# TU-Delft-AI-Energy-Lab/Deep-Statistical-Solver-for-Distribution-System-State-Estimation

Hardware: AMD Instinct MI355X
Metric: grid-samples/sec fwd+bwd (WLS loss), CIGRE-14 batch=4096, 1/2/4/8 GPU (higher is better)
Workload: dtype f32 (H->H products as f16x3: two fp16 pieces per operand, 3 fp16 MFMAs per fp32 product, f32 accumulate; edge MLP bf16x6; everything else f32/f64); 1 GPU; CIGRE-14 (15 buses, 14 closed branches) B=4096 graphs/GPU, MPN L=4 H=128 K=2 dropout=0: forward + gsp_wls_edge + backward; graphs_per_gpu=4096, global_batch=4096, parallelism=dp1, ranks_seen=1, arithmetic_route=f16x3, plan_launches=9, clock_ramp_steps_before_warmup=5740, mode=launch plan (dss2_plan_run)

## Files before the change

### deep-statistical-solver-for-distribution-system-state-estimation_amd/_lib.py

```python
from __future__ import annotations

import ctypes as C
import os
import subprocess

_HERE = os.path.dirname(os.path.abspath(__file__))
LIB_PATH = os.environ.get("DSS2_LIB", os.path.join(_HERE, "libdss2_hip.so"))

c_f32p = C.c_void_p
c_i32p = C.c_void_p


class PackDesc(C.Structure):
    _fields_ = [("src", C.c_void_p), ("dst", C.c_void_p), ("rows", C.c_int32), ("cols", C.c_int32),
                ("ld", C.c_int32), ("transpose", C.c_int32), ("koff", C.c_int32), ("kpad", C.c_int32),
                ("ncg", C.c_int32), ("joff", C.c_int32)]


class GemmPropArgs(C.Structure):
    _fields_ = [("X", C.c_void_p), ("ldx", C.c_int64), ("kreal", C.c_int32), ("kpad", C.c_int32),
                ("Bp", C.c_void_p), ("bias", C.c_void_p), ("rowscale", C.c_void_p),
                ("relu_src", C.c_void_p), ("ld_relu", C.c_int64),
                ("dmask", C.c_void_p), ("ld_dmask", C.c_int64),
                ("add_src", C.c_void_p), ("ld_add", C.c_int64),
# ... 280 lines not shown
    "dss2_wgrad": (C.c_int, [C.POINTER(WgradArgs), C.c_void_p]),
    "dss2_wgrad_batched": (C.c_int, [C.c_void_p, C.c_void_p, C.c_void_p, C.c_void_p, C.c_void_p, C.c_int64, C.c_int, C.c_void_p]),
    "dss2_reduce_slabs_multi": (C.c_int, [C.c_void_p, C.c_int, C.c_void_p]),
    "dss2_reduce_slabs": (C.c_int, [C.c_void_p, C.c_int, C.c_int64, C.c_void_p, C.c_int64, C.c_void_p]),
    "dss2_wls_loss_partials": (C.c_int, [C.POINTER(WlsArgs), C.c_void_p]),
    "dss2_wls_loss_grad": (C.c_int, [C.POINTER(WlsArgs), C.c_void_p]),
    "dss2_wls_loss_value": (C.c_int, [C.POINTER(WlsArgs), C.c_void_p]),
    "dss2_get_pflow": (C.c_int, [C.c_void_p, C.c_int64, C.c_void_p, C.c_int64, C.c_void_p, C.c_int64,
                                 C.c_void_p, C.c_void_p, C.c_int64, C.c_int64, C.c_void_p, C.c_void_p,
                                 C.c_int, C.c_void_p]),
    "dss2_eval_batch": (C.c_int, [C.c_void_p, C.c_int64, C.c_void_p, C.c_int64, C.c_void_p, C.c_int64, C.c_void_p, C.c_int64,
                                  C.c_void_p, C.c_void_p, C.c_int64, C.c_int64, C.c_void_p, C.c_void_p, C.c_void_p,
                                  C.c_void_p, C.c_void_p, C.c_void_p, C.c_void_p, C.c_void_p, C.c_void_p]),
    "dss2_eval_scratch_doubles": (C.c_int64, []),
    "dss2_small_gemm": (C.c_int, [C.c_void_p, C.c_int, C.c_int, C.c_void_p, C.c_void_p]),
    "dss2_measure_nodes": (C.c_int, [C.c_void_p, C.c_void_p, C.c_int32, C.c_void_p, C.c_double, C.c_double, C.c_double,
                                     C.c_double, C.c_void_p, C.c_int64, C.c_void_p]),
    "dss2_measure_edges": (C.c_int, [C.c_void_p, C.c_void_p, C.c_int32, C.c_void_p, C.c_double, C.c_void_p, C.c_int64,
                                     C.c_void_p]),
    "dss2_masked_zscore": (C.c_int, [C.c_void_p, C.c_int64, C.c_int32, C.c_int32, C.c_void_p, C.c_int32, C.c_void_p,
                                     C.c_void_p, C.c_void_p, C.c_void_p]),
    "dss2_masked_zscore_scratch_doubles": (C.c_int64, [C.c_int64]),
    "dss2_collate": (C.c_int, [C.c_void_p, C.c_int32, C.c_void_p, C.c_int64, C.c_void_p]),
    "dss2_csr_build_graphs": (C.c_int, [C.c_void_p, C.c_int32, C.c_void_p, C.c_int32, C.c_int32, C.c_void_p, C.c_void_p]),
    "dss2_csr_build_graphs_supported": (C.c_int, [C.c_int32, C.c_int32]),
    "dss2_csr_build_padded": (C.c_int, [C.POINTER(PaddedBuildArgs), C.c_void_p]),
    "dss2_collate_cursor": (C.c_int, [C.c_void_p, C.c_int32, C.c_void_p, C.c_void_p, C.c_int64, C.c_int, C.c_void_p]),
    "dss2_accum_scalar": (C.c_int, [C.c_void_p, C.c_void_p, C.c_void_p]),
    "dss2_collate_ragged_multi": (C.c_int, [C.c_void_p, C.c_int32, C.c_int32, C.c_void_p, C.c_void_p, C.c_void_p, C.c_void_p, C.c_int64, C.c_void_p]),
    "dss2_collate_ragged": (C.c_int, [C.c_void_p, C.c_int32, C.c_void_p, C.c_void_p, C.c_void_p, C.c_int64, C.c_int64, C.c_void_p]),
# ... 83 lines not shown
```

### deep-statistical-solver-for-distribution-system-state-estimation_amd/csrc/dss2_gemm_prop.hip

```cpp
#include <stdlib.h>

#include "dss2_weightspace.hpp"

namespace dss2 {

__global__ void __launch_bounds__(256) pack_weights_kernel(const dss2_pack_desc* __restrict__ descs) {
  pack_weights_body(descs[blockIdx.y], (int)blockIdx.x);
}

#ifdef DSS2_STAMPS
__device__ unsigned long long g_stamps[8192 * 8];
#define DSS2_STAMP(slot)                                                                       \
  do {                                                                                         \
    unsigned long long t_;                                                                     \
    __builtin_amdgcn_sched_barrier(0);                                                         \
    asm volatile("s_memtime %0\n\ts_waitcnt lgkmcnt(0)" : "=s"(t_)::"memory");                 \
    __builtin_amdgcn_sched_barrier(0);                                                         \
    if (lane == 0 && (stamp_tile * 4 + wave) < 8192) g_stamps[(stamp_tile * 4 + wave) * 8 + (slot)] = t_; \
  } while (0)
#define DSS2_STAMP2(slot)                                                                      \
  do {                                                                                         \
    unsigned long long t_;                                                                     \
    __builtin_amdgcn_sched_barrier(0);                                                         \
    asm volatile("s_memtime %0\n\ts_waitcnt lgkmcnt(0)" : "=s"(t_)::"memory");                 \
// ... 841 lines not shown

extern "C" size_t dss2_gemm_prop_lds_bytes(int nrb, int nmat, int kpad, int ncg, int max_nnz, int ell_width) {
  return dss2::lds_bytes(nrb, nmat, kpad, ncg, max_nnz, ell_width);
}

extern "C" int dss2_gemm_prop16_supported(int nrb, int nmat, int kreal, int hout, int max_nnz, int ell_width) {
  if (!((nrb == 6 && (nmat == 3 || nmat == 4)) || (nrb == 4 && nmat == 4))) return 0;
  return dss2::gemm16_shape_ok(nrb, nmat, kreal, hout, max_nnz, ell_width) ? 1 : 0;
}

static int dss2_pack_weights_launch(const dss2_pack_desc* descs, int n_desc, int max_elems, void* stream);
extern "C" int dss2_pack_weights(const dss2_pack_desc* descs, int n_desc, int max_elems, void* stream) {
  DSS2_RECORD([descs, n_desc, max_elems](void* s_) { return dss2_pack_weights_launch(descs, n_desc, max_elems, s_); });
  return dss2_pack_weights_launch(descs, n_desc, max_elems, stream);
}
static int dss2_pack_weights_launch(const dss2_pack_desc* descs, int n_desc, int max_elems, void* stream) {
  if (n_desc <= 0) return 0;
  dim3 grid((max_elems + 255) / 256, n_desc);
  hipLaunchKernelGGL(dss2::pack_weights_kernel, grid, dim3(256), 0, dss2::as_stream(stream), descs);
  return dss2::check_launch("pack_weights");
}

static int dss2_gemm_prop_launch(const dss2_gemm_prop_args* ap, void* stream);
extern "C" int dss2_gemm_prop(const dss2_gemm_prop_args* ap, void* stream) {
  if (!ap) { dss2::set_error("dss2_gemm_prop: null argument"); return 2; }
  DSS2_RECORD([a = *ap](void* s_) { return dss2_gemm_prop_launch(&a, s_); });
  return dss2_gemm_prop_launch(ap, stream);
}
static int dss2_gemm_prop_launch(const dss2_gemm_prop_args* ap, void* stream) {
  using namespace dss2;
// ... 63 lines not shown
```

### deep-statistical-solver-for-distribution-system-state-estimation_amd/csrc/dss2_weightspace.hpp

```cpp
#pragma once
#include "dss2_common.hpp"

namespace dss2 {

template <bool COH>
__device__ __forceinline__ void ws_store(float* p, float v) {
  if (COH) __hip_atomic_store((__attribute__((address_space(1))) float*)p, v, __ATOMIC_RELAXED, __HIP_MEMORY_SCOPE_AGENT);
  else *p = v;
}
template <bool COH>
__device__ __forceinline__ void ws_store4(float* p, f32x4 v) {
  if (COH) asm volatile("global_store_dwordx4 %0, %1, off sc1" ::"v"(p), "v"(v) : "memory");
  else *reinterpret_cast<f32x4*>(p) = v;
}

constexpr int SG_T = 32, SG_KC = 128, SG_LDA = SG_KC + 4;
template <bool tA, bool tB, bool COH = false, int NBUF = 3>
__device__ __forceinline__ void small_gemm_body(const dss2_sgemm_desc* __restrict__ dp, float* base_out,
                                                float (&As)[SG_T][SG_LDA], float (&Bs)[SG_KC][SG_T + 1], const int tile) {
  const int M = dp->M, N = dp->N, K = dp->K, lda = dp->lda, ldb = dp->ldb, ldc = dp->ldc;
  const bool accum = dp->accumulate != 0;
  const int nbatch = dp->nbatch;
  const float* u = dp->u;
  const float* v = dp->v;
  float* C = dp->c_off >= 0 ? base_out + dp->c_off : dp->C;
  const int tn = (N + SG_T - 1) / SG_T, tm = (M + SG_T - 1) / SG_T;
  if (tile >= tm * tn) return;
  const int i0 = (tile / tn) * SG_T, j0 = (tile % tn) * SG_T;
  const int t = threadIdx.x, lo = t & 31, hi = t >> 5;
  const int kchunks = (K + SG_KC - 1) / SG_KC;
  const int nchunks = nbatch * kchunks;
  float rab[NBUF][16], rbb[NBUF][16];
  auto issue = [&](int c, float (&ra)[16], float (&rb)[16]) {
    const int bidx = c / kchunks, k0 = (c - bidx * kchunks) * SG_KC;
    typedef const __attribute__((address_space(1))) float* gptr;
    const gptr A = (gptr)dp->A[bidx];
    const gptr B = (gptr)dp->B[bidx];
#pragma unroll
    for (int q = 0; q < 16; ++q) {
      const int i = tA ? lo : hi + 8 * (q >> 2), k = tA ? hi + 8 * q : lo + 32 * (q & 3);
      const int gi = min(i0 + i, M - 1), gk = min(k0 + k, K - 1);
      const float av = tA ? A[(size_t)gk * lda + gi] : A[(size_t)gi * lda + gk];
      ra[q] = av * (((i0 + i) < M && (k0 + k) < K) ? 1.f : 0.f);
      const int kb = tB ? lo + 32 * (q & 3) : hi + 8 * q, j = tB ? hi + 8 * (q >> 2) : lo;
      const int gj = min(j0 + j, N - 1), gkb = min(k0 + kb, K - 1);
      const float bv = tB ? B[(size_t)gj * ldb + gkb] : B[(size_t)gkb * ldb + gj];
      rb[q] = bv * (((j0 + j) < N && (k0 + kb) < K) ? 1.f : 0.f);
    }
// ... 20 lines not shown
      __syncthreads();
      stage(rab[u3], rbb[u3]);
      __syncthreads();
      if (c + NBUF < nchunks) issue(c + NBUF, rab[u3], rbb[u3]);
      const int kw = wave * 32;
#pragma unroll
      for (int g = 0; g < 8; ++g) {
        const f32x4 av = *reinterpret_cast<const f32x4*>(&As[c32][kw + 4 * g]);
#pragma unroll
        for (int tt = 0; tt < 2; ++tt) {
          const float a = half ? av[2 * tt + 1] : av[2 * tt];
          const float bvv = Bs[kw + 4 * g + 2 * tt + half][c32];
          acc = __builtin_amdgcn_mfma_f32_32x32x2f32(a, bvv, acc, 0, 0, 0);
        }
      }
    }
  }
  __syncthreads();
  float* red = &As[0][0];
#pragma unroll
  for (int r = 0; r < 16; ++r) red[(wave * 16 + r) * 64 + lane] = acc[r];
  __syncthreads();
  const int j = j0 + c32;
  if (j < N) {
    const float vj = u ? v[j] : 0.f;
#pragma unroll
    for (int q = 0; q < 4; ++q) {
      const int r = 4 * wave + q;
      const int i = i0 + (r & 3) + 8 * (r >> 2) + 4 * half;
      if (i >= M) continue;
      float sum = (red[(0 * 16 + r) * 64 + lane] + red[(1 * 16 + r) * 64 + lane]) + (red[(2 * 16 + r) * 64 + lane] + red[(3 * 16 + r) * 64 + lane]);
      if (u) sum = fmaf(u[i], vj, sum);
      float* cp = C + (size_t)i * ldc + j;
      ws_store<COH>(cp, accum ? *cp + sum : sum);
    }
  }
}

template <bool COH = false, int NBUF = 3>
__device__ __forceinline__ void small_gemm_tile(const dss2_sgemm_desc* __restrict__ dp, float* base_out,
                                                float (&As)[SG_T][SG_LDA], float (&Bs)[SG_KC][SG_T + 1], const int tile) {
  const bool ta = dp->transA != 0, tb = dp->transB != 0;
  if (ta) { if (tb) small_gemm_body<true, true, COH, NBUF>(dp, base_out, As, Bs, tile); else small_gemm_body<true, false, COH, NBUF>(dp, base_out, As, Bs, tile); }
  else    { if (tb) small_gemm_body<false, true, COH, NBUF>(dp, base_out, As, Bs, tile); else small_gemm_body<false, false, COH, NBUF>(dp, base_out, As, Bs, tile); }
}

__device__ __forceinline__ void pack_weights_body(const dss2_pack_desc d, const int bx) {
  const bool tr = d.transpose & 1;
  const int K = tr ? d.cols : d.rows;
  const int J = tr ? d.rows : d.cols;
  if (d.transpose & 8) {
    const int nkk = d.kpad >> 4, ncg = d.ncg;
    const int units = 2 * nkk;
    int U = 2; while (U < units) U <<= 1;
    if (U > 256) return;
    const int cpb = 256 / U;
    const int jpad = ncg * 32;
    if (bx * cpb >= jpad) return;
    __shared__ float cmx[256];
    typedef const __attribute__((address_space(1))) float* gsrc_t;
    const gsrc_t src = (gsrc_t)d.src;
    const int t = threadIdx.x, u = t & (U - 1), cj = t / U;
    const int j = bx * cpb + cj, kg = u >> 1, hf = u & 1;
    const bool active = u < units && j < jpad;
    float v[8];
    float mx = 0.f;
#pragma unroll
    for (int q = 0; q < 8; ++q) {
      const int k = kg * 16 + 8 * hf + q;
      const int kc = k >= K ? K - 1 : k, jc = j >= J ? J - 1 : j;
      const float x = tr ? src[(size_t)jc * d.ld + kc] : src[(size_t)kc * d.ld + jc];
      v[q] = (active && k < K && j < J) ? x : 0.f;
      mx = fmaxf(mx, fabsf(v[q]));
    }
// ... 58 lines not shown
  const int idx = bx * 256 + (int)threadIdx.x;
  if (idx >= total) return;
  const int lane = idx & 63;
  const int kg = kg0 + (idx >> 6) % nkl;
  const int cg = cg0 + (idx >> 6) / nkl;
  const int j = cg * 32 + (lane & 31) - d.joff;
  if (j < 0 || j >= J) return;
  float* dst = d.dst + (((size_t)cg * nkk + kg) * 64 + lane) * 4;
#pragma unroll
  for (int s = 0; s < 4; ++s) {
    const int k = kg * 8 + 4 * (lane >> 5) + s - d.koff;
    if (k >= 0 && k < K) dst[s] = tr ? d.src[(size_t)j * d.ld + k] : d.src[(size_t)k * d.ld + j];
  }
}


constexpr int REDUCE_MAX_DESC = 32;
struct ReduceTable { dss2_reduce_desc d[REDUCE_MAX_DESC]; uint32_t scalar_mask; };
__host__ __device__ __forceinline__ bool reduce_tall(const dss2_reduce_desc& d) { return d.n_slabs >= 256 && d.len <= 8192; }
__host__ __device__ __forceinline__ int64_t reduce_blocks(const dss2_reduce_desc& d, bool scalar) {
  return (!scalar && reduce_tall(d)) ? (d.len + 15) / 16 : (d.len + 63) / 64;
}
template <bool COH = false>
__device__ __forceinline__ void reduce_slabs_body(const dss2_reduce_desc& d, const bool scalar, const int bx, f32x4 (&part)[16][16]) {
  if (!scalar && reduce_tall(d)) {
    if ((int64_t)bx * 16 >= d.len) return;
    const int tid = threadIdx.x, cl = tid & 3, sl = tid >> 2;
    const int64_t i4 = (int64_t)bx * 16 + cl * 4;
    f32x4 s = {0.f, 0.f, 0.f, 0.f};
    f32x4* pt = &part[0][0];
// ... 88 lines not shown
```

### deep-statistical-solver-for-distribution-system-state-estimation_amd/flags.py

```python
import os as _os

EDGE_TILE_KERNELS = _os.environ.get("DSS2_EDGE_TILE", "1") == "1"
CHAIN_LAYERS = _os.environ.get("DSS2_CHAIN", "1") == "1"
WGRAD_BF16 = _os.environ.get("DSS2_WGRAD_BF16", "1") == "1"
CHAIN_GATE_BITS = _os.environ.get("DSS2_CHAIN_GATE_BITS", "1") == "1"
CHAIN_BF16 = _os.environ.get("DSS2_CHAIN_BF16", "1") == "1"
CHAIN_F16 = _os.environ.get("DSS2_CHAIN_F16", "1") == "1"
CHAIN_HEAD = _os.environ.get("DSS2_CHAIN_HEAD", "1") == "1"
CHAIN_HEAD_WGRAD = _os.environ.get("DSS2_CHAIN_HEAD_WGRAD", "1") == "1"
CHAIN_HEAD_FWD = _os.environ.get("DSS2_CHAIN_HEAD_FWD", "1") == "1"
CHAIN_EDGE = _os.environ.get("DSS2_CHAIN_EDGE", "1") == "1"
WGRAD_BATCH = _os.environ.get("DSS2_WGRAD_BATCH", "1") == "1"
STACK_NODE = _os.environ.get("DSS2_STACK_NODE", "1") == "1"
DX_MERGE = _os.environ.get("DSS2_DX_MERGE", "1") == "1"
WGRAD_JOIN_FOLDED = None
FOLD_W2 = _os.environ.get("DSS2_FOLD_W2", "1") == "1"
WGRAD_F16 = _os.environ.get("DSS2_WGRAD_F16", "1") == "1"
WGRAD_HOPS_MFMA = _os.environ.get("DSS2_WGRAD_HOPS_MFMA", "1") == "1"
WLS_FUSED_FINISH = _os.environ.get("DSS2_WLS_FUSED_FINISH", "0") == "1"
WLS_FUSED_FINISH_SMALL = _os.environ.get("DSS2_WLS_FUSED_FINISH_SMALL", "1") == "1"
WGRAD_TM32 = _os.environ.get("DSS2_WGRAD_TM32", "1") == "1"
WGRAD_TM32_MAX_BYTES = 64 << 20
WGRAD_PER_CU = int(_os.environ.get("DSS2_WGRAD_PER_CU", "2"))
CHAIN_MAX = 8
```

### deep-statistical-solver-for-distribution-system-state-estimation_amd/networks.py

```python
from __future__ import annotations

import ctypes as C
import os as _os
from typing import List, NamedTuple, Optional, Sequence, Tuple

import numpy as np
import torch
import torch.nn as nn

from . import _lib
from .topology import Topology, get_topology

_F32 = torch.float32

from . import flags as FL
from .ops import (_DROP_PARAMS, _dropout_params, _ncg, _ptr, _reduce, _require_gpu, _round16, _round8, _rows, _stream, _wgrad_per_cu, _wgrad_tiles, chain16_supported, chain_f16_supported, chain_gate_words, chain_edge_supported, chain_head_supported, chain_head_wgrad_supported, chain_supported, csr_axpy, dropout_mask, dropout_snapshot, edge_hidden_bwd, edge_hidden_fwd, edge_tile_bwd, edge_tile_fwd, gather_rows, gemm16_supported, gemm_prop, gemm_prop_chain, is_narrow, finish_weights, prep_weights, reduce_pending, segment_sum, wgrad, wgrad_batched)
from .plans import (_DESC_DTYPE, _FoldPlan, _MatView, _PackPlan, _SG_DTYPE, _as_view, _pack_table, _sg, _sg_table, _small_gemm)
from .route import BlockRoute, block_route, use_global_path


def _edge_aggr_forward(topo, x, ldx, ea, ldea, W1, b1, b2, pack_w2_fwd, hid, hout, fn, fe, second_linear=True, need_dx=False):
    N, ts = topo.N, topo.tiling
    S = torch.empty(N, hid, dtype=_F32, device=W1.device)
    if ts.ell_ent_tiles is not None and FL.EDGE_TILE_KERNELS:
        edge_tile_fwd(ts, x, ldx, ea, ldea, W1, b1, S, hid, fn, fe, need_dx)
    else:
        edge_hidden_fwd(topo, x, ldx, ea, ldea, W1, b1, S, hid, fn, fe)
    if not second_linear:
        return S, None
    x0 = torch.empty(N, hout, dtype=_F32, device=W1.device)
    gemm_prop(topo, S, hid, hid, pack_w2_fwd, 1, hout, x0, bias=b2, rowscale=topo.deg)
    return S, x0

# ... 488 lines not shown
    ver: int
    act_bits: dict


def _mpn_forward(mod, topo, x, ea, ps, stack=None, need_dx=False):
    x, ldx = _rows(x)
    ea, ldea = _rows(ea)
    dev = x.device
    L, nmat, hid = mod.n_gnn_layers, mod.K + 1, mod.dim_hid
    W1, b1, W2, b2 = ps[0:4]
    conv_ps = mod._conv_params(ps)
    rt = block_route(mod, topo, need_dx, False) if stack is None else stack.route_of(mod)
    ntiles = topo.tiling.ntiles
    plan, fold = _ensure_plans(mod, topo, dev, ps, rt)
    if stack is None:
        ver = plan.refresh(fold)
    else:
        ver = plan.version
    if not rt.glob:
        topo.lds_check(nmat, _round8(hid), _ncg(hid))
    if rt.edge:
        S = h = torch.empty(topo.N, hid, dtype=_F32, device=dev)
    else:
        S, h = _edge_aggr_forward(topo, x, ldx, ea, ldea, W1, b1, b2, plan.fwd[0], hid, hid, mod.dim_featn, mod.dim_feate,
                                  second_linear=fold is None, need_dx=need_dx)
    if fold is not None:
        h = S
    acts = [h]
    act_bits = {}
    p = float(mod.dropout_rate)
    if p <= 0.0:
# ... 203 lines not shown
        return (dx, None, None, None, *grads)


class _StackPlan:

    DROP_STRIDE = 64

    def __init__(self, blocks, device):
        self.blocks, self.device = list(blocks), device
        sizes = [int(m._flat_offsets()[-1]) for m in self.blocks]
        self.base = [0]
        for s in sizes:
            self.base.append(self.base[-1] + s)
        self.total = self.base[-1]
        self.key = None
        self.fold_fwd = self.fold_bwd = self.pack_tab = None
        self.table_builds = 0

    def refresh(self, topo, params, routes):
        plans = [_ensure_plans(m, topo, self.device, ps, rt) for m, ps, rt in zip(self.blocks, params, routes)]
        key = tuple((id(p), id(f), p.pointers(), f.pointers() if f is not None else None) for p, f in plans)
        if key != self.key:
            fwd, bwd, recs, max_elems = [], [], [], 0
            for b, (p, f) in enumerate(plans):
                if f is not None:
                    f_, b_ = f.records(self.base[b])
                    fwd += f_
                    bwd += b_
                recs += p.records()
                max_elems = max(max_elems, p.max_elems)
            self.fold_fwd = _sg_table(fwd, self.device) if fwd else None
            self.fold_bwd = _sg_table(bwd, self.device) if bwd else None
            t, cnt, n_dep = _pack_table(recs, self.device)
            self.pack_tab = (t, cnt, max_elems, n_dep)
            self.key = key
            self.table_builds += 1
        prep_weights(self.fold_fwd, self.pack_tab, self.device)
        for p, _ in plans:
            p.version += 1


class _StackRun:

    def __init__(self, plan: _StackPlan, snapshot, routes):
        self.plan, self.snapshot, self.routes = plan, snapshot, routes

    def route_of(self, mod) -> BlockRoute:
        return self.routes[self.plan.blocks.index(mod)]

    def drop_base(self, mod) -> int:
        return self.plan.blocks.index(mod) * _StackPlan.DROP_STRIDE

# ... 98 lines not shown
```

### deep-statistical-solver-for-distribution-system-state-estimation_amd/ops.py

```python
from __future__ import annotations

import ctypes as C
import math
from typing import Optional, Sequence, Tuple

import torch
import torch.nn as nn

from . import _lib
from . import flags as FL
from .topology import Tiling, Topology


def _static_replay() -> bool:
    from .graphs import plan_recording
    return plan_recording() or torch.cuda.is_current_stream_capturing()


_F32 = torch.float32


def _stream(t: torch.Tensor) -> int:
    return _lib.stream_ptr(t.device)

# ... 323 lines not shown
    descs = (_lib.ReduceDesc * len(chunk))()
    for d, (slab, ptr, n_slabs, stride, out, length) in zip(descs, chunk):
        d.slab, d.out, d.stride, d.len, d.n_slabs = ptr, out.data_ptr(), stride, length, n_slabs
    return descs


def reduce_pending(pending) -> None:
    for c0 in range(0, len(pending), 32):
        chunk = pending[c0:c0 + 32]
        descs = _reduce_descs(chunk)
        _lib.check(_lib.lib().dss2_reduce_slabs_multi(C.addressof(descs), len(chunk), _stream(chunk[0][0])),
                   "dss2_reduce_slabs_multi")
    pending.clear()


def prep_weights(fold_tab, pack_tab, device) -> None:
    t, cnt, mx, _n_dep = pack_tab
    st = _lib.stream_ptr(device)
    if fold_tab is not None:
        ft, fcnt, fmx = fold_tab
        _lib.check(_lib.lib().dss2_small_gemm(ft.data_ptr(), fcnt, fmx, None, st), "dss2_small_gemm")
    _lib.check(_lib.lib().dss2_pack_weights(t.data_ptr(), cnt, mx, st), "dss2_pack_weights")


def finish_weights(pending, rule_tab, base: Optional[torch.Tensor], device) -> None:
    if pending:
        reduce_pending(pending)
    if rule_tab is None:
        return
    rt, rcnt, rmx = rule_tab
    _lib.check(_lib.lib().dss2_small_gemm(rt.data_ptr(), rcnt, rmx, base.data_ptr(), _lib.stream_ptr(device)), "dss2_small_gemm")


# ... 118 lines not shown
```

### deep-statistical-solver-for-distribution-system-state-estimation_amd/plans.py

```python
from __future__ import annotations

import ctypes as C
from typing import List, Optional, Sequence

import numpy as np
import torch

from . import _lib
from . import flags as FL
from .ops import _F32, _ncg, _round8, _round16, is_narrow, prep_weights

_DESC_DTYPE = np.dtype([("src", "<u8"), ("dst", "<u8"), ("rows", "<i4"), ("cols", "<i4"), ("ld", "<i4"),
                        ("transpose", "<i4"), ("koff", "<i4"), ("kpad", "<i4"), ("ncg", "<i4"), ("joff", "<i4")])


_SG_DTYPE = np.dtype([("A", "<u8", (4,)), ("B", "<u8", (4,)), ("C", "<u8"), ("u", "<u8"), ("v", "<u8"), ("c_off", "<i8"),
                      ("M", "<i4"), ("N", "<i4"), ("K", "<i4"), ("lda", "<i4"), ("ldb", "<i4"), ("ldc", "<i4"),
                      ("transA", "<i4"), ("transB", "<i4"), ("nbatch", "<i4"), ("accumulate", "<i4")])


def _sg(A, B, M, N, K, lda, ldb, ldc, C=0, c_off=-1, tA=0, tB=0, u=0, v=0):
    A = list(A) + [0] * (4 - len(A))
    B = list(B) + [0] * (4 - len(B))
    nb = sum(1 for a in A if a)
    return (A, B, C, u, v, c_off, M, N, K, lda, ldb, ldc, tA, tB, nb, 0)


def _sg_table(recs, device):
    arr = np.zeros(len(recs), dtype=_SG_DTYPE)
    for i, r in enumerate(recs):
        arr[i] = tuple(r)
    return (torch.from_numpy(arr.view(np.uint8).copy()).to(device), len(recs),
            max(((r[6] + 31) // 32) * ((r[7] + 31) // 32) for r in recs))


def _pack_table(recs, device):
    recs = sorted(recs, key=lambda r: 0 if (r[5] & 4) else 1)
    arr = np.array(recs, dtype=_DESC_DTYPE)
    return torch.from_numpy(arr.view(np.uint8).copy()).to(device), len(recs), sum(1 for r in recs if r[5] & 4)


def _small_gemm(tab, base, device) -> None:
    t, cnt, mx = tab
    _lib.check(_lib.lib().dss2_small_gemm(t.data_ptr(), cnt, mx, base, _lib.stream_ptr(device)), "dss2_small_gemm")


class _FoldPlan:

    def __init__(self, W2, b2, ws, device, off_w2: int, off_conv0: int):
        nm, (ho, hid) = len(ws), ws[0].shape
        self.nm, self.ho, self.hid, self.device = nm, ho, hid, device
        self.Wf = torch.zeros(nm, ho, hid, dtype=_F32, device=device)
        self.bf = torch.zeros(nm, ho, dtype=_F32, device=device)
        self.gfold = torch.zeros(nm * ho * hid + ho + nm * ho, dtype=_F32, device=device)
# ... 10 lines not shown
        off_conv0, off_w2 = self.off_conv0 + base_off, self.off_w2 + base_off
        for m, w in enumerate(ws):
            fwd.append(_sg([w.data_ptr()], [W2.data_ptr()], ho, hid, hid, hid, hid, hid, C=self.Wf[m].data_ptr()))
            fwd.append(_sg([w.data_ptr()], [b2.data_ptr()], ho, 1, hid, hid, 1, 1, C=self.bf[m].data_ptr()))
        g = self.gfold.data_ptr()
        dWf = [g + f4 * m * ho * hid for m in range(nm)]
        db = g + f4 * nm * ho * hid
        dbf = [db + f4 * ho + f4 * m * ho for m in range(nm)]
        for m, w in enumerate(ws):
            bwd.append(_sg([dWf[m]], [W2.data_ptr()], ho, hid, hid, hid, hid, hid, c_off=off_conv0 + m * ho * hid,
                           tB=1, u=dbf[m], v=b2.data_ptr()))
        bwd.append(_sg([], [], ho, 1, 0, 1, 1, 1, c_off=off_conv0 + nm * ho * hid, u=db, v=self.one.data_ptr()))
        bwd.append(_sg([w.data_ptr() for w in ws], dWf, hid, hid, ho, hid, hid, hid, c_off=off_w2, tA=1))
        bwd.append(_sg([w.data_ptr() for w in ws], dbf, hid, 1, ho, hid, 1, 1, c_off=off_w2 + hid * hid, tA=1))
        return fwd, bwd

    def _tables(self):
        fwd, bwd = self.records()
        self.fwd_tab, self.bwd_tab = _sg_table(fwd, self.device), _sg_table(bwd, self.device)

    def pointers(self):
        W2, b2, ws = self.params
        return (W2.data_ptr(), b2.data_ptr()) + tuple(w.data_ptr() for w in ws)

    def _check(self):
        ptrs = self.pointers()
        if ptrs != self.ptrs:
            self._tables()
            self.ptrs = ptrs

# ... 47 lines not shown
                kf, cf, kb, cb = _round8(hin), _ncg(hout), _round8(hout), _ncg(hin)
                self.fwd.append(torch.zeros(nm * cf * (kf // 8) * 256, dtype=_F32, device=device))
                self.bwd.append(torch.zeros(nm * cb * (kb // 8) * 256, dtype=_F32, device=device))
            self.meta.append((nm, hout, hin, kf, cf, kb, cb))
        self.fwd16, self.bwd16, self.f16 = {}, {}, bool(f16)
        for g in bf16_groups:
            nm, hout, hin = self.meta[g][0:3]
            if is_narrow(nm, hout) or self._stk[g]:
                raise ValueError("bf16x3 packing is for plain per-matrix layouts")
            kf, cf, kb, cb = _round16(hin), _ncg(hout), _round16(hout), _ncg(hin)
            per = 512 if self.f16 else 768
            self.fwd16[g] = torch.zeros(nm * cf * (kf // 16) * per + (nm * cf * 32 if self.f16 else 0), dtype=_F32, device=device)
            self.bwd16[g] = torch.zeros(nm * cb * (kb // 16) * per + (nm * cb * 32 if self.f16 else 0), dtype=_F32, device=device)
        self.ptrs = None
        self.table = None
        self.max_elems = 0
        self.version = 0

    def pointers(self):
        return tuple(w.data_ptr() for mats in self.groups for w in mats)

    def records(self):
        recs = []
        for g, mats in enumerate(self.groups):
            nm, hout, hin, kf, cf, kb, cb = self.meta[g]
            narrow = is_narrow(nm, hout) or self._stk[g]
            for m, w in enumerate(mats):
                if not w.is_contiguous():
                    raise RuntimeError("weight matrices must be contiguous")
                dp = 4 if w.dep else 0
# ... 5 lines not shown
                    recs.append((w.data_ptr(), self.bwd[g].data_ptr() + 4 * m * cb * (kb // 8) * 256, hout, hin, w.ld, 0 | dp, 0, kb, cb, 0))
                self.max_elems = max(self.max_elems, (cf + 1) * (kf // 8 + 1) * 64, (cb + 1) * (kb // 8 + 1) * 64)
                if g in self.fwd16 and self.f16:
                    k16, b16 = _round16(hin), _round16(hout)
                    recs.append((w.data_ptr(), self.fwd16[g].data_ptr(), hout, hin, w.ld, 9 | dp, nm, k16, cf, m))
                    recs.append((w.data_ptr(), self.bwd16[g].data_ptr(), hout, hin, w.ld, 8 | dp, nm, b16, cb, m))
                elif g in self.fwd16:
                    k16, b16 = _round16(hin), _round16(hout)
                    recs.append((w.data_ptr(), self.fwd16[g].data_ptr() + 4 * m * cf * (k16 // 16) * 768, hout, hin, w.ld, 3 | dp, 0, k16, cf, 0))
                    recs.append((w.data_ptr(), self.bwd16[g].data_ptr() + 4 * m * cb * (b16 // 16) * 768, hout, hin, w.ld, 2 | dp, 0, b16, cb, 0))
        return recs

    def _build_table(self):
        self.table, self.n_desc, self.n_dep = _pack_table(self.records(), self.device)

    def refresh(self, fold: Optional["_FoldPlan"] = None):
        ptrs = self.pointers()
        if ptrs != self.ptrs:
            self._build_table()
            self.ptrs = ptrs
        fold_tab = None
        if fold is not None:
            fold._check()
            fold_tab = fold.fwd_tab
        prep_weights(fold_tab, (self.table, self.n_desc, self.max_elems, self.n_dep), self.device)
        self.version += 1
        return self.version
```

### deep-statistical-solver-for-distribution-system-state-estimation_amd/route.py

```python
from __future__ import annotations

from typing import NamedTuple, Tuple

from . import flags as FL
from .ops import (_tiles, chain16_supported, chain_edge_supported, chain_f16_supported, chain_gate_words, chain_head_supported,
                  chain_head_wgrad_supported, chain_supported, gemm16_supported, is_narrow)
from .topology import Topology


def use_global_path(topo: Topology, nmat: int) -> bool:
    return bool(_tiles(topo).global_only or nmat > 4)


class BlockRoute(NamedTuple):
    glob: bool
    fold: bool
    b16: Tuple[int, ...]
    f16: bool
    n_chain: int
    use16: bool
    gw: int
    head: bool
    edge: bool
    g16: Tuple[bool, ...]
# ... 34 lines not shown
    bwd_use16 = bool(bwd_chain and b16 and chain16_supported(topo, nmat, hid, True))
    bwd_head = bool(bwd_use16 and L - 1 <= FL.CHAIN_MAX and narrow_head and chain_head_supported(topo, nmat, hid, nout, True)
                    and (_tiles(topo).nrb <= 2 or gw > 0))
    bwd_head_wgrad = bool(bwd_head and chain_head_wgrad_supported(topo, nmat, hid, nout))
    bwd_edge = bool(bwd_head and edge_ok and chain_edge_supported(topo, nmat, hid, True))
    bwd_join = bool(bwd_chain and fold and L - 1 <= 8 and (FL.WGRAD_JOIN_FOLDED is None or FL.WGRAD_JOIN_FOLDED))
    if bwd_chain:
        bwd_g16 = (False,) * L
        bwd_defer = tuple(not bwd_join and (1 if fold else 0) <= l < L - 1 for l in range(L))
    else:
        bwd_g16 = tuple(tall16(l, True) for l in range(L))
        bwd_defer = tuple(bool(FL.WGRAD_BATCH and not glob and not (l == 0 and fold) and houts[l] == hid and not is_narrow(nmat, hid))
                          for l in range(L))
    return BlockRoute(glob, fold, b16, f16, n_chain, use16, gw, head, edge, g16,
                      bwd_chain, bwd_use16, bwd_head, bwd_head_wgrad, bwd_edge, bwd_join, bwd_g16, bwd_defer)
```

### include/dss2_hip.h

```cpp
#ifndef DSS2_HIP_H
#define DSS2_HIP_H

#include <stddef.h>
#include <stdint.h>

#ifdef __cplusplus
extern "C" {
#endif

const char* dss2_last_error(void);
int dss2_version(void);


int dss2_topology_probe(const int64_t* edge_index, int64_t n_edges, uint64_t* out3, void* stream);

typedef struct dss2_plan dss2_plan;
int dss2_plan_begin(dss2_plan** out);
int dss2_plan_end(dss2_plan* plan);
int dss2_plan_size(const dss2_plan* plan);
int dss2_plan_run(const dss2_plan* plan, void* stream);
void dss2_plan_destroy(dss2_plan* plan);

typedef struct dss2_csr_build_args {
  const int64_t* edge_index; int64_t n_edges; int64_t n_nodes; int32_t doubled;
// ... 238 lines not shown
int dss2_eval_batch(const float* out, int64_t ldo, const float* y, int64_t ldy, const float* node_param, int64_t ld_np,
                    const float* edge_param, int64_t ld_ep, const int32_t* efrom, const int32_t* eto,
                    int64_t n_nodes, int64_t n_edges, const float* x_mean, const float* x_std, float* yhat,
                    float* pf_true, float* pf_out, float* vminmax, double* scratch, double* acc, void* stream);
int64_t dss2_eval_scratch_doubles(void);

typedef struct dss2_sgemm_desc {
  const float* A[4]; const float* B[4];
  float* C;
  const float* u; const float* v;
  int64_t c_off;
  int32_t M, N, K, lda, ldb, ldc, transA, transB, nbatch, accumulate;
} dss2_sgemm_desc;

int dss2_small_gemm(const dss2_sgemm_desc* descs, int n_desc, int max_tiles, float* base_out, void* stream);


int dss2_measure_nodes(const double* nodes, const uint8_t* meas_v_mask, int32_t n_per_sample, const double* z,
                       double v_noise, double pm_noise, double p_noise, double zero_inj_coef, float* x, int64_t rows,
                       void* stream);

int dss2_measure_edges(const double* edges, const uint8_t* meas_pflow_mask, int32_t e_per_sample, const double* z,
                       double p_noise, float* edge_attr, int64_t rows, void* stream);

int dss2_masked_zscore(const float* t, int64_t rows, int32_t ld, int32_t num_feat, float* out, int32_t ld_out,
                       float* mean, float* stdv, double* scratch, void* stream);
int64_t dss2_masked_zscore_scratch_doubles(int64_t rows);

typedef struct dss2_collate_desc {
  const void* src; void* dst;
// ... 203 lines not shown
```

Baseline: 11.60 million graphs/s.

## Fuse weight-fold small GEMM into weight packing kernel

Adds a fold_pack kernel that computes each folded weight product strip in LDS and then packs it directly into the split-precision MFMA layout. This replaces the separate small_gemm launch plus pack_weights launch, so the folded weights no longer round-trip through global memory. The small_gemm core is refactored into a generic product with an emit callback, and independent pack records and vector products share the same grid. In exchange, each block recomputes a full column strip serially across tiles, which lowers parallelism inside the fused kernel and needs more LDS.

```diff
diff --git a/deep-statistical-solver-for-distribution-system-state-estimation_amd/_lib.py b/deep-statistical-solver-for-distribution-system-state-estimation_amd/_lib.py
--- a/deep-statistical-solver-for-distribution-system-state-estimation_amd/_lib.py
+++ b/deep-statistical-solver-for-distribution-system-state-estimation_amd/_lib.py
@@ -318,6 +318,7 @@
                                   C.c_void_p, C.c_void_p, C.c_void_p, C.c_void_p, C.c_void_p, C.c_void_p]),
     "dss2_eval_scratch_doubles": (C.c_int64, []),
     "dss2_small_gemm": (C.c_int, [C.c_void_p, C.c_int, C.c_int, C.c_void_p, C.c_void_p]),
+    "dss2_fold_pack": (C.c_int, [C.c_void_p, C.c_int, C.c_int, C.c_void_p, C.c_int, C.c_int, C.c_void_p]),
     "dss2_measure_nodes": (C.c_int, [C.c_void_p, C.c_void_p, C.c_int32, C.c_void_p, C.c_double, C.c_double, C.c_double,
                                      C.c_double, C.c_void_p, C.c_int64, C.c_void_p]),
     "dss2_measure_edges": (C.c_int, [C.c_void_p, C.c_void_p, C.c_int32, C.c_void_p, C.c_double, C.c_void_p, C.c_int64,
diff --git a/deep-statistical-solver-for-distribution-system-state-estimation_amd/csrc/dss2_gemm_prop.hip b/deep-statistical-solver-for-distribution-system-state-estimation_amd/csrc/dss2_gemm_prop.hip
--- a/deep-statistical-solver-for-distribution-system-state-estimation_amd/csrc/dss2_gemm_prop.hip
+++ b/deep-statistical-solver-for-distribution-system-state-estimation_amd/csrc/dss2_gemm_prop.hip
@@ -5,7 +5,21 @@
 namespace dss2 {
 
 __global__ void __launch_bounds__(256) pack_weights_kernel(const dss2_pack_desc* __restrict__ descs) {
-  pack_weights_body(descs[blockIdx.y], (int)blockIdx.x);
+  __shared__ float cmx[256];
+  pack_weights_body(descs[blockIdx.y], (int)blockIdx.x, cmx);
+}
+
+constexpr size_t FOLD_PACK_LDS = sizeof(float) * (SG_T * SG_LDA + SG_KC * (SG_T + 1) + FP_KMAX * FP_LDS);
+__global__ void __launch_bounds__(256) fold_pack_kernel(const dss2_pack_desc* __restrict__ descs, const dss2_sgemm_desc* __restrict__ sg,
+                                                        const int n_dep, const int n_pack) {
+  extern __shared__ __attribute__((aligned(16))) float fp_lds[];
+  float (&As)[SG_T][SG_LDA] = *reinterpret_cast<float (*)[SG_T][SG_LDA]>(fp_lds);
+  float (&Bs)[SG_KC][SG_T + 1] = *reinterpret_cast<float (*)[SG_KC][SG_T + 1]>(fp_lds + SG_T * SG_LDA);
+  float (*W)[FP_LDS] = reinterpret_cast<float (*)[FP_LDS]>(fp_lds + SG_T * SG_LDA + SG_KC * (SG_T + 1));
+  const int y = blockIdx.y;
+  if (y < n_dep) fold_pack_body(descs[y], sg + y, (int)blockIdx.x, As, Bs, W);
+  else if (y < n_pack) pack_weights_body(descs[y], (int)blockIdx.x, &As[0][0]);
+  else small_gemm_tile(sg + n_dep + (y - n_pack), nullptr, As, Bs, (int)blockIdx.x);
 }
 
 #ifdef DSS2_STAMPS
@@ -879,6 +893,19 @@
   DSS2_RECORD([descs, n_desc, max_elems](void* s_) { return dss2_pack_weights_launch(descs, n_desc, max_elems, s_); });
   return dss2_pack_weights_launch(descs, n_desc, max_elems, stream);
 }
+static int dss2_fold_pack_launch(const dss2_pack_desc* descs, int n_pack, int n_dep, const dss2_sgemm_desc* sg, int n_vec, int grid_x, void* stream);
+extern "C" int dss2_fold_pack(const dss2_pack_desc* descs, int n_pack, int n_dep, const dss2_sgemm_desc* sg, int n_vec, int grid_x, void* stream) {
+  DSS2_RECORD([descs, n_pack, n_dep, sg, n_vec, grid_x](void* s_) { return dss2_fold_pack_launch(descs, n_pack, n_dep, sg, n_vec, grid_x, s_); });
+  return dss2_fold_pack_launch(descs, n_pack, n_dep, sg, n_vec, grid_x, stream);
+}
+static int dss2_fold_pack_launch(const dss2_pack_desc* descs, int n_pack, int n_dep, const dss2_sgemm_desc* sg, int n_vec, int grid_x, void* stream) {
+  if (n_pack <= 0) return 0;
+  if (n_dep < 0 || n_dep > n_pack || n_vec < 0 || grid_x <= 0 || ((n_dep > 0 || n_vec > 0) && !sg)) { dss2::set_error("fold_pack: inconsistent table sizes"); return 2; }
+  static std::atomic<uint32_t> lds_done{0};
+  if (dss2::ensure_max_lds(reinterpret_cast<const void*>(dss2::fold_pack_kernel), lds_done, "fold_pack")) return 1;
+  hipLaunchKernelGGL(dss2::fold_pack_kernel, dim3(grid_x, n_pack + n_vec), dim3(256), dss2::FOLD_PACK_LDS, dss2::as_stream(stream), descs, sg, n_dep, n_pack);
+  return dss2::check_launch("fold_pack");
+}
 static int dss2_pack_weights_launch(const dss2_pack_desc* descs, int n_desc, int max_elems, void* stream) {
   if (n_desc <= 0) return 0;
   dim3 grid((max_elems + 255) / 256, n_desc);
diff --git a/deep-statistical-solver-for-distribution-system-state-estimation_amd/csrc/dss2_weightspace.hpp b/deep-statistical-solver-for-distribution-system-state-estimation_amd/csrc/dss2_weightspace.hpp
--- a/deep-statistical-solver-for-distribution-system-state-estimation_amd/csrc/dss2_weightspace.hpp
+++ b/deep-statistical-solver-for-distribution-system-state-estimation_amd/csrc/dss2_weightspace.hpp
@@ -15,23 +15,35 @@
 }
 
 constexpr int SG_T = 32, SG_KC = 128, SG_LDA = SG_KC + 4;
-template <bool tA, bool tB, bool COH = false, int NBUF = 3>
-__device__ __forceinline__ void small_gemm_body(const dss2_sgemm_desc* __restrict__ dp, float* base_out,
-                                                float (&As)[SG_T][SG_LDA], float (&Bs)[SG_KC][SG_T + 1], const int tile) {
-  const int M = dp->M, N = dp->N, K = dp->K, lda = dp->lda, ldb = dp->ldb, ldc = dp->ldc;
-  const bool accum = dp->accumulate != 0;
+template <bool tA, bool tB, int NBUF, class Emit>
+__device__ __forceinline__ void small_gemm_product(const dss2_sgemm_desc* __restrict__ dp, float (&As)[SG_T][SG_LDA], float (&Bs)[SG_KC][SG_T + 1],
+                                                   const int tile0, const int tile_stride, const int nseq, Emit emit) {
+  const int M = dp->M, N = dp->N, K = dp->K, lda = dp->lda, ldb = dp->ldb;
   const int nbatch = dp->nbatch;
-  const float* u = dp->u;
-  const float* v = dp->v;
-  float* C = dp->c_off >= 0 ? base_out + dp->c_off : dp->C;
-  const int tn = (N + SG_T - 1) / SG_T, tm = (M + SG_T - 1) / SG_T;
-  if (tile >= tm * tn) return;
-  const int i0 = (tile / tn) * SG_T, j0 = (tile % tn) * SG_T;
+  const int tn = (N + SG_T - 1) / SG_T;
+  if (nseq <= 0) return;
   const int t = threadIdx.x, lo = t & 31, hi = t >> 5;
   const int kchunks = (K + SG_KC - 1) / SG_KC;
-  const int nchunks = nbatch * kchunks;
+  const int per_tile = nbatch * kchunks;
+  const int nchunks = nseq * per_tile;
+  if (per_tile == 0) {
+    const int w_ = t >> 6, l_ = t & 63;
+    for (int q_ = 0; q_ < nseq; ++q_) {
+      const int tile = tile0 + q_ * tile_stride;
+      const int j = (tile % tn) * SG_T + (l_ & 31);
+      for (int q = 0; q < 4; ++q) {
+        const int r = 4 * w_ + q;
+        const int i = (tile / tn) * SG_T + (r & 3) + 8 * (r >> 2) + 4 * (l_ >> 5);
+        if (i < M && j < N) emit(i, j, 0.f);
+      }
+    }
+    return;
+  }
   float rab[NBUF][16], rbb[NBUF][16];
-  auto issue = [&](int c, float (&ra)[16], float (&rb)[16]) {
+  auto issue = [&](int cc, float (&ra)[16], float (&rb)[16]) {
+    const int q_ = cc / per_tile, c = cc - q_ * per_tile;
+    const int tile = tile0 + q_ * tile_stride;
+    const int i0 = (tile / tn) * SG_T, j0 = (tile % tn) * SG_T;
     const int bidx = c / kchunks, k0 = (c - bidx * kchunks) * SG_KC;
     typedef const __attribute__((address_space(1))) float* gptr;
     const gptr A = (gptr)dp->A[bidx];
@@ -82,27 +94,42 @@
           acc = __builtin_amdgcn_mfma_f32_32x32x2f32(a, bvv, acc, 0, 0, 0);
         }
       }
-    }
-  }
-  __syncthreads();
-  float* red = &As[0][0];
-#pragma unroll
-  for (int r = 0; r < 16; ++r) red[(wave * 16 + r) * 64 + lane] = acc[r];
-  __syncthreads();
-  const int j = j0 + c32;
-  if (j < N) {
-    const float vj = u ? v[j] : 0.f;
-#pragma unroll
-    for (int q = 0; q < 4; ++q) {
-      const int r = 4 * wave + q;
-      const int i = i0 + (r & 3) + 8 * (r >> 2) + 4 * half;
-      if (i >= M) continue;
-      float sum = (red[(0 * 16 + r) * 64 + lane] + red[(1 * 16 + r) * 64 + lane]) + (red[(2 * 16 + r) * 64 + lane] + red[(3 * 16 + r) * 64 + lane]);
-      if (u) sum = fmaf(u[i], vj, sum);
-      float* cp = C + (size_t)i * ldc + j;
-      ws_store<COH>(cp, accum ? *cp + sum : sum);
-    }
-  }
+      if ((c + 1) % per_tile != 0) continue;
+      __syncthreads();
+      float* red = &As[0][0];
+#pragma unroll
+      for (int r = 0; r < 16; ++r) { red[(wave * 16 + r) * 64 + lane] = acc[r]; acc[r] = 0.f; }
+      __syncthreads();
+      const int tile = tile0 + (c / per_tile) * tile_stride;
+      const int i0 = (tile / tn) * SG_T, j0 = (tile % tn) * SG_T;
+      const int j = j0 + c32;
+      if (j < N) {
+#pragma unroll
+        for (int q = 0; q < 4; ++q) {
+          const int r = 4 * wave + q;
+          const int i = i0 + (r & 3) + 8 * (r >> 2) + 4 * half;
+          if (i >= M) continue;
+          emit(i, j, (red[(0 * 16 + r) * 64 + lane] + red[(1 * 16 + r) * 64 + lane]) + (red[(2 * 16 + r) * 64 + lane] + red[(3 * 16 + r) * 64 + lane]));
+        }
+      }
+    }
+  }
+}
+
+template <bool tA, bool tB, bool COH = false, int NBUF = 3>
+__device__ __forceinline__ void small_gemm_body(const dss2_sgemm_desc* __restrict__ dp, float* base_out,
+                                                float (&As)[SG_T][SG_LDA], float (&Bs)[SG_KC][SG_T + 1], const int tile) {
+  const int M = dp->M, N = dp->N, ldc = dp->ldc;
+  if (tile >= ((M + SG_T - 1) / SG_T) * ((N + SG_T - 1) / SG_T)) return;
+  const bool accum = dp->accumulate != 0;
+  const float* u = dp->u;
+  const float* v = dp->v;
+  float* C = dp->c_off >= 0 ? base_out + dp->c_off : dp->C;
+  small_gemm_product<tA, tB, NBUF>(dp, As, Bs, tile, 0, 1, [&](int i, int j, float sum) {
+    if (u) sum = fmaf(u[i], v[j], sum);
+    float* cp = C + (size_t)i * ldc + j;
+    ws_store<COH>(cp, accum ? *cp + sum : sum);
+  });
 }
 
 template <bool COH = false, int NBUF = 3>
@@ -113,7 +140,7 @@
   else    { if (tb) small_gemm_body<false, true, COH, NBUF>(dp, base_out, As, Bs, tile); else small_gemm_body<false, false, COH, NBUF>(dp, base_out, As, Bs, tile); }
 }
 
-__device__ __forceinline__ void pack_weights_body(const dss2_pack_desc d, const int bx) {
+__device__ __forceinline__ void pack_weights_body(const dss2_pack_desc d, const int bx, float* cmx) {
   const bool tr = d.transpose & 1;
   const int K = tr ? d.cols : d.rows;
   const int J = tr ? d.rows : d.cols;
@@ -125,7 +152,6 @@
     const int cpb = 256 / U;
     const int jpad = ncg * 32;
     if (bx * cpb >= jpad) return;
-    __shared__ float cmx[256];
     typedef const __attribute__((address_space(1))) float* gsrc_t;
     const gsrc_t src = (gsrc_t)d.src;
     const int t = threadIdx.x, u = t & (U - 1), cj = t / U;
@@ -214,6 +240,92 @@
   }
 }
 
+constexpr int FP_KMAX = 256, FP_LDS = SG_T + 1;
+__device__ __forceinline__ void fold_pack_body(const dss2_pack_desc d, const dss2_sgemm_desc* __restrict__ prod, const int strip,
+                                               float (&As)[SG_T][SG_LDA], float (&Bs)[SG_KC][SG_T + 1], float (*W)[FP_LDS]) {
+  const bool tr = d.transpose & 1;
+  const int K = tr ? d.cols : d.rows;
+  const int J = tr ? d.rows : d.cols;
+  if (strip >= d.ncg || K > FP_KMAX) return;
+  const int jb = strip * SG_T;
+  const int M = prod->M, N = prod->N;
+  if (M != d.rows || N != d.cols) return;
+  const int tn = (N + SG_T - 1) / SG_T, tm = (M + SG_T - 1) / SG_T;
+  if (jb < J) {
+    const bool ta = prod->transA != 0, tb = prod->transB != 0;
+    const int tile0 = tr ? strip * tn : strip, stride = tr ? 1 : tn, nseq = tr ? tn : tm;
+    auto emit = [&](int i, int j, float sum) { if (tr) W[j][i - jb] = sum; else W[i][j - jb] = sum; };
+    if (ta) { if (tb) small_gemm_product<true, true, 3>(prod, As, Bs, tile0, stride, nseq, emit); else small_gemm_product<true, false, 3>(prod, As, Bs, tile0, stride, nseq, emit); }
+    else    { if (tb) small_gemm_product<false, true, 3>(prod, As, Bs, tile0, stride, nseq, emit); else small_gemm_product<false, false, 3>(prod, As, Bs, tile0, stride, nseq, emit); }
+  }
+  __syncthreads();
+  const int t = threadIdx.x;
+  if (d.transpose & 8) {
+    const int nkk = d.kpad >> 4, units = 2 * nkk, jpad = d.ncg * 32;
+    float* cmx = &As[0][0];
+    const int c = t & 31, kl = t >> 5, j = jb + c;
+    float mx = 0.f;
+    if (j < J) for (int k = kl; k < K; k += 8) mx = fmaxf(mx, fabsf(W[k][c]));
+    cmx[kl * 32 + c] = mx;
+    __syncthreads();
+    float cm = 0.f;
+#pragma unroll
+    for (int w = 0; w < 8; ++w) cm = fmaxf(cm, cmx[w * 32 + c]);
+    const int s = cm > 0.f ? 14 - exp_of(cm) : 0;
+    const size_t mat_bytes = (size_t)d.ncg * nkk * 2048;
+    char* gb = reinterpret_cast<char*>(d.dst);
+    if (kl == 0) reinterpret_cast<int*>(gb + (size_t)d.koff * mat_bytes)[(size_t)d.joff * jpad + j] = s;
+    typedef __attribute__((address_space(1))) uint32_t* gdst_t;
+    for (int u = kl; u < units; u += 8) {
+      const int kg = u >> 1, hf = u & 1, lane = hf * 32 + c;
+      float v[8];
+#pragma unroll
+      for (int q = 0; q < 8; ++q) {
+        const int k = kg * 16 + 8 * hf + q;
+        v[q] = (k < K && j < J) ? W[k < K ? k : 0][c] : 0.f;
+      }
+      gdst_t dst = (gdst_t)(gb + (size_t)d.joff * mat_bytes + (((size_t)strip * nkk + kg) * 2 * 64 + lane) * 16);
+#pragma unroll
+      for (int q = 0; q < 4; ++q) {
+        uint32_t h, l;
+        split2_pair(ldexpf(v[2 * q], s), ldexpf(v[2 * q + 1], s), h, l);
+        dst[q] = h; dst[64 * 4 + q] = l;
+      }
+    }
+    return;
+  }
+  if (jb >= J) return;
+  if (d.transpose & 2) {
+    const int nkk = d.kpad >> 4, nkl = (K + 15) >> 4;
+    typedef __attribute__((address_space(1))) __bf16* gdst_t;
+    for (int idx = t; idx < nkl * 64; idx += 256) {
+      const int lane = idx & 63, kg = idx >> 6, c = lane & 31;
+      if (jb + c >= J) continue;
+      gdst_t dst = (gdst_t)(reinterpret_cast<__bf16*>(d.dst) + (((size_t)strip * nkk + kg) * 3 * 64 + lane) * 8);
+#pragma unroll
+      for (int q = 0; q < 8; ++q) {
+        const int k = kg * 16 + 8 * (lane >> 5) + q;
+        if (k >= K) continue;
+        __bf16 h, m, l;
+        split3(W[k][c], h, m, l);
+        dst[q] = h; dst[64 * 8 + q] = m; dst[2 * 64 * 8 + q] = l;
+      }
+    }
+    return;
+  }
+  const int nkk = d.kpad >> 3, nkl = (K + 7) >> 3;
+  for (int idx = t; idx < nkl * 64; idx += 256) {
+    const int lane = idx & 63, kg = idx >> 6, c = lane & 31;
+    if (jb + c >= J) continue;
+    float* dst = d.dst + (((size_t)strip * nkk + kg) * 64 + lane) * 4;
+#pragma unroll
+    for (int q = 0; q < 4; ++q) {
+      const int k = kg * 8 + 4 * (lane >> 5) + q;
+      if (k < K) dst[q] = W[k][c];
+    }
+  }
+}
+
 
 constexpr int REDUCE_MAX_DESC = 32;
 struct ReduceTable { dss2_reduce_desc d[REDUCE_MAX_DESC]; uint32_t scalar_mask; };
diff --git a/deep-statistical-solver-for-distribution-system-state-estimation_amd/flags.py b/deep-statistical-solver-for-distribution-system-state-estimation_amd/flags.py
--- a/deep-statistical-solver-for-distribution-system-state-estimation_amd/flags.py
+++ b/deep-statistical-solver-for-distribution-system-state-estimation_amd/flags.py
@@ -15,6 +15,7 @@
 DX_MERGE = _os.environ.get("DSS2_DX_MERGE", "1") == "1"
 WGRAD_JOIN_FOLDED = None
 FOLD_W2 = _os.environ.get("DSS2_FOLD_W2", "1") == "1"
+FOLD_IN_PACK = _os.environ.get("DSS2_FOLD_IN_PACK", "1") == "1"
 WGRAD_F16 = _os.environ.get("DSS2_WGRAD_F16", "1") == "1"
 WGRAD_HOPS_MFMA = _os.environ.get("DSS2_WGRAD_HOPS_MFMA", "1") == "1"
 WLS_FUSED_FINISH = _os.environ.get("DSS2_WLS_FUSED_FINISH", "0") == "1"
diff --git a/deep-statistical-solver-for-distribution-system-state-estimation_amd/networks.py b/deep-statistical-solver-for-distribution-system-state-estimation_amd/networks.py
--- a/deep-statistical-solver-for-distribution-system-state-estimation_amd/networks.py
+++ b/deep-statistical-solver-for-distribution-system-state-estimation_amd/networks.py
@@ -15,8 +15,9 @@
 
 from . import flags as FL
 from .ops import (_DROP_PARAMS, _dropout_params, _ncg, _ptr, _reduce, _require_gpu, _round16, _round8, _rows, _stream, _wgrad_per_cu, _wgrad_tiles, chain16_supported, chain_f16_supported, chain_gate_words, chain_edge_supported, chain_head_supported, chain_head_wgrad_supported, chain_supported, csr_axpy, dropout_mask, dropout_snapshot, edge_hidden_bwd, edge_hidden_fwd, edge_tile_bwd, edge_tile_fwd, gather_rows, gemm16_supported, gemm_prop, gemm_prop_chain, is_narrow, finish_weights, prep_weights, reduce_pending, segment_sum, wgrad, wgrad_batched)
-from .plans import (_DESC_DTYPE, _FoldPlan, _MatView, _PackPlan, _SG_DTYPE, _as_view, _pack_table, _sg, _sg_table, _small_gemm)
-from .route import BlockRoute, block_route, use_global_path
+from .plans import (_DESC_DTYPE, _FoldPlan, _MatView, _PackPlan, _SG_DTYPE, _as_view, _fold_pack_table, _pack_table, _sg, _sg_table,
+                    _small_gemm)
+from .route import BlockRoute, block_route, fold_in_pack, use_global_path
 
 
 def _edge_aggr_forward(topo, x, ldx, ea, ldea, W1, b1, b2, pack_w2_fwd, hid, hout, fn, fe, second_linear=True, need_dx=False):
@@ -535,7 +536,7 @@
     ntiles = topo.tiling.ntiles
     plan, fold = _ensure_plans(mod, topo, dev, ps, rt)
     if stack is None:
-        ver = plan.refresh(fold)
+        ver = plan.refresh(fold, fold_in_pack(mod, rt))
     else:
         ver = plan.version
     if not rt.glob:
@@ -769,7 +770,7 @@
             self.base.append(self.base[-1] + s)
         self.total = self.base[-1]
         self.key = None
-        self.fold_fwd = self.fold_bwd = self.pack_tab = None
+        self.fold_fwd = self.fold_bwd = self.pack_tab = self.fused = None
         self.table_builds = 0
 
     def refresh(self, topo, params, routes):
@@ -788,9 +789,11 @@
             self.fold_bwd = _sg_table(bwd, self.device) if bwd else None
             t, cnt, n_dep = _pack_table(recs, self.device)
             self.pack_tab = (t, cnt, max_elems, n_dep)
+            self.fused = _fold_pack_table(recs, [f for _, f in plans if f is not None], max_elems, self.device) if fwd else None
             self.key = key
             self.table_builds += 1
-        prep_weights(self.fold_fwd, self.pack_tab, self.device)
+        in_pack = self.fused is not None and all(fold_in_pack(m, rt) for m, rt in zip(self.blocks, routes) if rt.fold)
+        prep_weights(self.fold_fwd, self.pack_tab, self.device, self.fused if in_pack else None)
         for p, _ in plans:
             p.version += 1
 
diff --git a/deep-statistical-solver-for-distribution-system-state-estimation_amd/ops.py b/deep-statistical-solver-for-distribution-system-state-estimation_amd/ops.py
--- a/deep-statistical-solver-for-distribution-system-state-estimation_amd/ops.py
+++ b/deep-statistical-solver-for-distribution-system-state-estimation_amd/ops.py
@@ -361,9 +361,13 @@
     pending.clear()
 
 
-def prep_weights(fold_tab, pack_tab, device) -> None:
+def prep_weights(fold_tab, pack_tab, device, fused=None) -> None:
+    st = _lib.stream_ptr(device)
+    if fused is not None:
+        t, cnt, n_dep, sg, n_vec, grid_x = fused
+        _lib.check(_lib.lib().dss2_fold_pack(t.data_ptr(), cnt, n_dep, sg.data_ptr(), n_vec, grid_x, st), "dss2_fold_pack")
+        return
     t, cnt, mx, _n_dep = pack_tab
-    st = _lib.stream_ptr(device)
     if fold_tab is not None:
         ft, fcnt, fmx = fold_tab
         _lib.check(_lib.lib().dss2_small_gemm(ft.data_ptr(), fcnt, fmx, None, st), "dss2_small_gemm")
diff --git a/deep-statistical-solver-for-distribution-system-state-estimation_amd/plans.py b/deep-statistical-solver-for-distribution-system-state-estimation_amd/plans.py
--- a/deep-statistical-solver-for-distribution-system-state-estimation_amd/plans.py
+++ b/deep-statistical-solver-for-distribution-system-state-estimation_amd/plans.py
@@ -38,6 +38,23 @@
     recs = sorted(recs, key=lambda r: 0 if (r[5] & 4) else 1)
     arr = np.array(recs, dtype=_DESC_DTYPE)
     return torch.from_numpy(arr.view(np.uint8).copy()).to(device), len(recs), sum(1 for r in recs if r[5] & 4)
+
+
+def _fold_pack_table(recs, folds, max_elems, device):
+    prods, vecs = {}, []
+    for f in folds:
+        p_, v_ = f.fused_records()
+        prods.update(p_)
+        vecs += v_
+    recs = sorted(recs, key=lambda r: 0 if (r[5] & 4) else 1)
+    dep = [r for r in recs if r[5] & 4]
+    for r in dep:
+        if r[0] not in prods or ((r[6] or r[9]) and not r[5] & 8):
+            raise RuntimeError("fold_pack: a dependent packing record without its product, or with an offset")
+    sg = [prods[r[0]] for r in dep] + vecs
+    arr = np.array(recs, dtype=_DESC_DTYPE)
+    grid_x = max([(max_elems + 255) // 256] + [r[8] for r in dep] + [((v[6] + 31) // 32) * ((v[7] + 31) // 32) for v in vecs])
+    return (torch.from_numpy(arr.view(np.uint8).copy()).to(device), len(recs), len(dep), _sg_table(sg, device)[0], len(vecs), grid_x)
 
 
 def _small_gemm(tab, base, device) -> None:
@@ -78,6 +95,10 @@
         bwd.append(_sg([w.data_ptr() for w in ws], dWf, hid, hid, ho, hid, hid, hid, c_off=off_w2, tA=1))
         bwd.append(_sg([w.data_ptr() for w in ws], dbf, hid, 1, ho, hid, 1, 1, c_off=off_w2 + hid * hid, tA=1))
         return fwd, bwd
+
+    def fused_records(self):
+        fwd = self.records()[0]
+        return {self.Wf[m].data_ptr(): fwd[2 * m] for m in range(self.nm)}, [fwd[2 * m + 1] for m in range(self.nm)]
 
     def _tables(self):
         fwd, bwd = self.records()
@@ -155,6 +176,7 @@
             self.bwd16[g] = torch.zeros(nm * cb * (kb // 16) * per + (nm * cb * 32 if self.f16 else 0), dtype=_F32, device=device)
         self.ptrs = None
         self.table = None
+        self.fused, self.fused_key = None, None
         self.max_elems = 0
         self.version = 0
 
@@ -190,15 +212,20 @@
     def _build_table(self):
         self.table, self.n_desc, self.n_dep = _pack_table(self.records(), self.device)
 
-    def refresh(self, fold: Optional["_FoldPlan"] = None):
+    def refresh(self, fold: Optional["_FoldPlan"] = None, in_pack: bool = False):
         ptrs = self.pointers()
         if ptrs != self.ptrs:
             self._build_table()
             self.ptrs = ptrs
-        fold_tab = None
+        fold_tab = fused = None
         if fold is not None:
             fold._check()
             fold_tab = fold.fwd_tab
-        prep_weights(fold_tab, (self.table, self.n_desc, self.max_elems, self.n_dep), self.device)
+            if in_pack:
+                key = (ptrs, fold.pointers())
+                if key != self.fused_key:
+                    self.fused, self.fused_key = _fold_pack_table(self.records(), [fold], self.max_elems, self.device), key
+                fused = self.fused
+        prep_weights(fold_tab, (self.table, self.n_desc, self.max_elems, self.n_dep), self.device, fused)
         self.version += 1
         return self.version
diff --git a/deep-statistical-solver-for-distribution-system-state-estimation_amd/route.py b/deep-statistical-solver-for-distribution-system-state-estimation_amd/route.py
--- a/deep-statistical-solver-for-distribution-system-state-estimation_amd/route.py
+++ b/deep-statistical-solver-for-distribution-system-state-estimation_amd/route.py
@@ -72,3 +72,11 @@
                           for l in range(L))
     return BlockRoute(glob, fold, b16, f16, n_chain, use16, gw, head, edge, g16,
                       bwd_chain, bwd_use16, bwd_head, bwd_head_wgrad, bwd_edge, bwd_join, bwd_g16, bwd_defer)
+
+
+FOLD_PACK_MAX_DIM = 256
+
+
+def fold_in_pack(mod, rt: BlockRoute) -> bool:
+    ho = mod.dim_out if mod.n_gnn_layers == 1 else mod.dim_hid
+    return bool(rt.fold and FL.FOLD_IN_PACK and max(mod.dim_hid, ho) <= FOLD_PACK_MAX_DIM)
diff --git a/include/dss2_hip.h b/include/dss2_hip.h
--- a/include/dss2_hip.h
+++ b/include/dss2_hip.h
@@ -276,6 +276,8 @@
 } dss2_sgemm_desc;
 
 int dss2_small_gemm(const dss2_sgemm_desc* descs, int n_desc, int max_tiles, float* base_out, void* stream);
+
+int dss2_fold_pack(const dss2_pack_desc* descs, int n_pack, int n_dep, const dss2_sgemm_desc* sg, int n_vec, int grid_x, void* stream);
 
 
 int dss2_measure_nodes(const double* nodes, const uint8_t* meas_v_mask, int32_t n_per_sample, const double* z,
```

Measured after the change: 11.30 million graphs/s. 2.5% lower.
